# truongp-aws/neuronx-distributed-llama3_2

Hardware: AMD Instinct MI355X
Metric: tokens/sec (whole node) Llama-3-8B TP=8 bf16 training at 1/2/4/8 MI355X (higher is better)
Workload: dtype bf16

## Files before the change

### neuronx_distributed_llama3_2_amd/csrc/dense_gemm.hip

```cpp
#include "gemm_tile.h"

#include <cstdlib>
#include <type_traits>

namespace nxd {
namespace dg {

constexpr int BM = 256, BN = 256, BK = 64, NT = 512;
constexpr int REG = 16384;
constexpr int BUF = 4 * REG;
constexpr int LDS_BYTES = 2 * BUF;
constexpr int R_ALO = 0, R_AHI = REG, R_BLO = 2 * REG, R_BHI = 3 * REG;

enum Layout { LNT = 0, LTN = 1 };
enum Epi { BF16 = 0, F32_ACC = 1, F32_ATOMIC = 2 };

struct Params {
  const uint16_t* a;
  const uint16_t* b;
  void* c;
  int M, N, K;
  int64_t lda, ldb, ldc;
  int mt, nt;
  int splits;
  int k_per_split;
  int band;
};

__device__ __forceinline__ int nt_swz(int r) { return (r >> 1) & 7; }

__device__ __forceinline__ bf16x8_t frag_nt(const char* reg, int r0, int s) {
  const int l = threadIdx.x & 63, r = r0 + (l & 15), ch = (l >> 4) + 4 * s;
  return __builtin_bit_cast(bf16x8_t, *reinterpret_cast<const u32x4_t*>(reg + r * 128 + ((ch ^ nt_swz(r)) << 4)));
}
template <int L>
__device__ __forceinline__ bf16x8_t frag(const char* reg, int x0, int s) {
  if constexpr (L == LNT) return frag_nt(reg, x0, s);
  else return frag_tr16<256>(reg, x0, 32 * s);
}

__device__ __forceinline__ void wait_regions(int younger) {
  switch (younger) {
    case 5: asm volatile("s_waitcnt vmcnt(10)" ::: "memory"); break;
    case 4: asm volatile("s_waitcnt vmcnt(8)" ::: "memory"); break;
    case 3: asm volatile("s_waitcnt vmcnt(6)" ::: "memory"); break;
    case 2: asm volatile("s_waitcnt vmcnt(4)" ::: "memory"); break;
    case 1: asm volatile("s_waitcnt vmcnt(2)" ::: "memory"); break;
    default: asm volatile("s_waitcnt vmcnt(0)" ::: "memory"); break;
  }
}

template <int L, int E>
__global__ void __launch_bounds__(NT, 1) gemm_kernel(Params p) {
  __shared__ __attribute__((aligned(16))) char smem[LDS_BYTES];
  const int tiles = p.mt * p.nt;
  const int id = xcd_remap(blockIdx.x, gridDim.x);
  const int split = id / tiles;
  int rt, ct;
  band_raster(id - split * tiles, p.mt, p.nt, p.band, rt, ct);
  const int m0 = rt * BM, n0 = ct * BN;
  const int k_begin = split * p.k_per_split;
  const int k_end = min(p.K, k_begin + p.k_per_split);
  const int nk = (k_end - k_begin) / BK;

  const int wid = threadIdx.x >> 6, lane = threadIdx.x & 63;
  const int wr = wid >> 2, wc = wid & 3;

  f32x4_t acc[4][4][2];
#pragma unroll
  for (int q = 0; q < 4; ++q)
#pragma unroll
    for (int i = 0; i < 4; ++i)
#pragma unroll
      for (int j = 0; j < 2; ++j) acc[q][i][j] = f32x4_t{0.f, 0.f, 0.f, 0.f};

  const uint16_t* sa[2][2];
  const uint16_t* sb[2][2];
#pragma unroll
  for (int h = 0; h < 2; ++h)
#pragma unroll
    for (int j = 0; j < 2; ++j) {
      const int piece = 2 * wid + j;
      if constexpr (L == LNT) {
        const int pr = 8 * piece + (lane >> 3), c = (lane & 7) ^ nt_swz(pr);
        sa[h][j] = p.a + (int64_t)min(m0 + 128 * h + pr, p.M - 1) * p.lda + k_begin + 8 * c;
        sb[h][j] = p.b + (int64_t)min(n0 + 128 * h + pr, p.N - 1) * p.ldb + k_begin + 8 * c;
      } else {
        const int pr = 4 * piece + (lane >> 4), c = (lane & 15) ^ tok_swz(pr);
        sa[h][j] = p.a + (int64_t)(k_begin + pr) * p.lda + min(m0 + 128 * h + 8 * c, p.M - 8);
        sb[h][j] = p.b + (int64_t)(k_begin + pr) * p.ldb + min(n0 + 128 * h + 8 * c, p.N - 8);
      }
    }
  const int64_t adv_a = L == LNT ? (int64_t)BK : (int64_t)BK * p.lda;
  const int64_t adv_b = L == LNT ? (int64_t)BK : (int64_t)BK * p.ldb;
  const uint32_t lds0 = lds_addr(smem);

  auto issue = [&](auto rc, int s) {
    constexpr int R = decltype(rc)::value;
    if (s >= nk) return;
    const uint32_t dst = lds0 + (s & 1) * BUF + (R == 0 ? R_ALO : R == 1 ? R_BLO : R == 2 ? R_BHI : R_AHI) + wid * 2048;
    if constexpr (R == 0 || R == 3) {
      constexpr int h = R == 0 ? 0 : 1;
      const int64_t o = (int64_t)s * adv_a;
      dma16(sa[h][0] + o, __builtin_amdgcn_readfirstlane(dst));
      dma16(sa[h][1] + o, __builtin_amdgcn_readfirstlane(dst + 1024));
    } else {
      constexpr int h = R == 1 ? 0 : 1;
      const int64_t o = (int64_t)s * adv_b;
      dma16(sb[h][0] + o, __builtin_amdgcn_readfirstlane(dst));
      dma16(sb[h][1] + o, __builtin_amdgcn_readfirstlane(dst + 1024));
    }
  };
  const int last = 4 * nk - 1;
  auto wait_for = [&](int need, int max_younger = 4) {
    if (need > last) return;
    wait_regions(min(max_younger, last - need));
  };

  using I0 = std::integral_constant<int, 0>;
  using I1 = std::integral_constant<int, 1>;
  using I2 = std::integral_constant<int, 2>;
  using I3 = std::integral_constant<int, 3>;
  bf16x8_t af[4][2], blo[2][2], bhi[2][2];

  issue(I0{}, 0); issue(I1{}, 0); issue(I2{}, 0); issue(I3{}, 0); issue(I0{}, 1); issue(I1{}, 1); issue(I2{}, 1);
  wait_for(1, 5);
  barrier();
#pragma unroll
  for (int i = 0; i < 4; ++i)
#pragma unroll
    for (int s = 0; s < 2; ++s) af[i][s] = frag<L>(smem + R_ALO, wr * 64 + 16 * i, s);
#pragma unroll
  for (int j = 0; j < 2; ++j)
#pragma unroll
    for (int s = 0; s < 2; ++s) blo[j][s] = frag<L>(smem + R_BLO, wc * 32 + 16 * j, s);
  wait_for(2);
  barrier();
  for (int t = 0; t < nk; ++t) {
    const char* buf = smem + (t & 1) * BUF;
    const char* nbuf = smem + ((t + 1) & 1) * BUF;
    issue(I3{}, t + 1);
#pragma unroll
    for (int s = 0; s < 2; ++s)
#pragma unroll
      for (int i = 0; i < 4; ++i) {
#pragma unroll
        for (int j = 0; j < 2; ++j)
          acc[0][i][j] = __builtin_amdgcn_mfma_f32_16x16x32_bf16(af[i][s], blo[j][s], acc[0][i][j], 0, 0, 0);
        if (i < 2) bhi[i][s] = frag<L>(buf + R_BHI, wc * 32 + 16 * i, s);
      }
    wait_for(4 * t + 3);
    barrier();
    issue(I0{}, t + 2);
#pragma unroll
    for (int s = 0; s < 2; ++s)
#pragma unroll
      for (int i = 0; i < 4; ++i) {
#pragma unroll
        for (int j = 0; j < 2; ++j)
          acc[1][i][j] = __builtin_amdgcn_mfma_f32_16x16x32_bf16(af[i][s], bhi[j][s], acc[1][i][j], 0, 0, 0);
        af[i][s] = frag<L>(buf + R_AHI, wr * 64 + 16 * i, s);
      }
    barrier();
    issue(I1{}, t + 2);
#pragma unroll
    for (int s = 0; s < 2; ++s)
#pragma unroll
      for (int i = 0; i < 4; ++i)
#pragma unroll
        for (int j = 0; j < 2; ++j)
          acc[2][i][j] = __builtin_amdgcn_mfma_f32_16x16x32_bf16(af[i][s], bhi[j][s], acc[2][i][j], 0, 0, 0);
    wait_for(4 * t + 5);
    barrier();
    issue(I2{}, t + 2);
#pragma unroll
    for (int s = 0; s < 2; ++s)
#pragma unroll
      for (int j = 0; j < 2; ++j) {
#pragma unroll
        for (int i = 0; i < 4; ++i) {
          acc[3][i][j] = __builtin_amdgcn_mfma_f32_16x16x32_bf16(af[i][s], blo[j][s], acc[3][i][j], 0, 0, 0);
          if (j == 1) af[i][s] = frag<L>(nbuf + R_ALO, wr * 64 + 16 * i, s);
        }
        blo[j][s] = frag<L>(nbuf + R_BLO, wc * 32 + 16 * j, s);
      }
    wait_for(4 * t + 6);
    barrier();
  }
  asm volatile("s_waitcnt vmcnt(0)" ::: "memory");
  __syncthreads();

  constexpr int LD = 36;
  float* slab = reinterpret_cast<float*>(smem) + wid * (64 * LD);
  const int crow = 4 * (lane >> 4), ccol = lane & 15;
#pragma unroll
  for (int qd = 0; qd < 4; ++qd) {
    const int rh = (qd == 2 || qd == 3) ? 1 : 0, ch = (qd == 1 || qd == 2) ? 1 : 0;
#pragma unroll
    for (int i = 0; i < 4; ++i)
#pragma unroll
      for (int j = 0; j < 2; ++j)
#pragma unroll
        for (int r = 0; r < 4; ++r) slab[(16 * i + crow + r) * LD + 16 * j + ccol] = acc[qd][i][j][r];
    __builtin_amdgcn_wave_barrier();
    const int row0 = m0 + 128 * rh + 64 * wr, col0 = n0 + 128 * ch + 32 * wc;
    if constexpr (E == F32_ATOMIC) {
      const int col = col0 + (lane & 31);
      float* cp = static_cast<float*>(p.c);
#pragma unroll 8
      for (int rr = 0; rr < 32; ++rr) {
        const int lr = 2 * rr + (lane >> 5), row = row0 + lr;
        const float v = slab[lr * LD + (lane & 31)];
        if (row < p.M && col < p.N) unsafeAtomicAdd(cp + (int64_t)row * p.ldc + col, v);
      }
    } else {
#pragma unroll
      for (int ps = 0; ps < 4; ++ps) {
        const int lr = 16 * ps + (lane >> 2), c8 = 8 * (lane & 3);
        const int row = row0 + lr, col = col0 + c8;
        const f32x4_t v0 = *reinterpret_cast<const f32x4_t*>(slab + lr * LD + c8);
        const f32x4_t v1 = *reinterpret_cast<const f32x4_t*>(slab + lr * LD + c8 + 4);
        if (row < p.M && col < p.N) {
          if constexpr (E == BF16) {
            u32x4_t o;
            o[0] = pack2bf(v0[0], v0[1]); o[1] = pack2bf(v0[2], v0[3]);
            o[2] = pack2bf(v1[0], v1[1]); o[3] = pack2bf(v1[2], v1[3]);
            *reinterpret_cast<u32x4_t*>(static_cast<uint16_t*>(p.c) + (int64_t)row * p.ldc + col) = o;
          } else {
            f32x4_t* cp = reinterpret_cast<f32x4_t*>(static_cast<float*>(p.c) + (int64_t)row * p.ldc + col);
            const f32x4_t c0 = cp[0], c1 = cp[1];
            cp[0] = c0 + v0;
            cp[1] = c1 + v1;
          }
        }
      }
    }
    __builtin_amdgcn_wave_barrier();
  }
}

static int env_int(const char* name, int dflt) {
  const char* e = getenv(name);
  return e ? atoi(e) : dflt;
}

}

int dense_gemm_choose_splits(int M, int N, int K) {
  const int tiles = ceil_div(M, dg::BM) * ceil_div(N, dg::BN);
  const int steps = K / dg::BK;
  const int64_t base = (int64_t)ceil_div(tiles, 256) * steps;
  int best = 1;
  int64_t best_cost = base;
  for (int s = 2; s <= 8 && s <= steps; ++s) {
    if (steps / s < 8) break;
    const int64_t cost = (int64_t)ceil_div(tiles * s, 256) * (ceil_div(steps, s) + 6);
    if (cost * 10 < best_cost * 9 && cost < best_cost) {
      best_cost = cost;
      best = s;
    }
  }
  return best;
}

int dense_gemm_launch(int layout, int epi, const void* a, int64_t lda, const void* b, int64_t ldb, void* c, int64_t ldc,
                      int M, int N, int K, int splits, hipStream_t stream) {
  if (M <= 0 || N <= 0 || K <= 0) return 0;
  if (K % dg::BK || N % 8 || lda % 8 || ldb % 8 || ldc % 4) return -1;
  if (layout == dg::LTN && M % 8) return -1;
  if (epi == dg::BF16 && ldc % 8) return -1;
  dg::Params p{};
  p.a = static_cast<const uint16_t*>(a);
  p.b = static_cast<const uint16_t*>(b);
  p.c = c;
  p.M = M; p.N = N; p.K = K;
  p.lda = lda; p.ldb = ldb; p.ldc = ldc;
  p.mt = ceil_div(M, dg::BM);
  p.nt = ceil_div(N, dg::BN);
  const int steps = K / dg::BK;
  if (epi != dg::F32_ATOMIC) splits = 1;
  else if (splits <= 0) splits = dense_gemm_choose_splits(M, N, K);
  splits = splits < 1 ? 1 : (splits > steps ? steps : splits);
  p.k_per_split = ceil_div(steps, splits) * dg::BK;
  p.splits = ceil_div(K, p.k_per_split);
  static const int band = [] { const int v = dg::env_int("NXD_DG_BAND", 8); return v > 0 ? v : 8; }();
  p.band = band;
  const int64_t nwg = (int64_t)p.mt * p.nt * p.splits;
  if (nwg > INT32_MAX) return -2;
#define NXD_DG_LAUNCH(LY, EP) \
  hipLaunchKernelGGL((dg::gemm_kernel<LY, EP>), dim3((unsigned)nwg), dim3(dg::NT), 0, stream, p)
  if (layout == dg::LNT) {
    if (epi == dg::BF16) NXD_DG_LAUNCH(dg::LNT, dg::BF16);
    else if (epi == dg::F32_ACC) NXD_DG_LAUNCH(dg::LNT, dg::F32_ACC);
    else NXD_DG_LAUNCH(dg::LNT, dg::F32_ATOMIC);
  } else {
    if (epi == dg::BF16) NXD_DG_LAUNCH(dg::LTN, dg::BF16);
    else if (epi == dg::F32_ACC) NXD_DG_LAUNCH(dg::LTN, dg::F32_ACC);
    else NXD_DG_LAUNCH(dg::LTN, dg::F32_ATOMIC);
  }
#undef NXD_DG_LAUNCH
  return hipGetLastError() == hipSuccess ? 0 : -3;
}

}
```

### neuronx_distributed_llama3_2_amd/csrc/gemm_tile.h

```cpp
#pragma once
#include "common.h"

namespace nxd {

typedef __attribute__((address_space(3))) char lds_char_t;
typedef __attribute__((address_space(3))) short4_t lds_short4_t;

__device__ __forceinline__ uint32_t lds_addr(const char* q) { return (uint32_t)(uintptr_t)(const lds_char_t*)q; }

__device__ __forceinline__ void dma16(const void* src, uint32_t lds_dst) {
  uint32_t sv;
  asm volatile("s_mov_b32 %0, m0\n\ts_mov_b32 m0, %2\n\ts_nop 0\n\tglobal_load_lds_dwordx4 %1, off\n\ts_mov_b32 m0, %0"
               : "=&s"(sv) : "v"(src), "s"(lds_dst) : "memory");
}

__device__ __forceinline__ void barrier() {
  __builtin_amdgcn_sched_barrier(0);
  __builtin_amdgcn_s_barrier();
  __builtin_amdgcn_sched_barrier(0);
}

__device__ __forceinline__ void band_raster(int id, int rows, int cols, int band, int& r, int& c) {
  const int bnd = id / (band * cols), within = id - bnd * band * cols;
  const int h = min(band, rows - bnd * band);
  r = bnd * band + within % h;
  c = within / h;
}

__device__ __forceinline__ int tok_swz(int t) { return 2 * ((t & 3) | (((t >> 3) & 1) << 2)); }

template <int PITCH>
__device__ __forceinline__ bf16x8_t frag_tr16(const char* img, int c0, int t0) {
  const int l = threadIdx.x & 63, g = l >> 4, i = l & 15, q = i >> 2, p = i & 3;
  const int col = c0 + 4 * p, t = t0 + 8 * g + q;
  const char* b0 = img + t * PITCH + 16 * ((col >> 3) ^ tok_swz(t)) + 8 * (p & 1);
  const char* b1 = img + (t + 4) * PITCH + 16 * ((col >> 3) ^ tok_swz(t + 4)) + 8 * (p & 1);
  const short4_t lo = __builtin_amdgcn_ds_read_tr16_b64_v4i16((lds_short4_t*)b0);
  const short4_t hi = __builtin_amdgcn_ds_read_tr16_b64_v4i16((lds_short4_t*)b1);
  const short __attribute__((ext_vector_type(8))) a8 = {lo[0], lo[1], lo[2], lo[3], hi[0], hi[1], hi[2], hi[3]};
  return __builtin_bit_cast(bf16x8_t, a8);
}

}
```

### neuronx_distributed_llama3_2_amd/ops/gemm.py

```python

from __future__ import annotations

import os

import torch

from ._ext import ext, use_native

_ENABLED = os.environ.get("NXD_TUNED_GEMM", "1") == "1"


def set_overlap_safe(enabled: bool) -> None:
    if not torch.cuda.is_available():
        return
    try:
        ext().gemm_set_no_streamk(1 if enabled else 0)
    except Exception:
        pass


def _native(*t: torch.Tensor) -> bool:
    return _ENABLED and use_native(*t) and all(x.dtype in (torch.bfloat16, torch.float16) for x in t)


def linear(x: torch.Tensor, w: torch.Tensor, bias=None, out: torch.Tensor = None) -> torch.Tensor:
    shape = x.shape[:-1] + (w.shape[0],)
    if _native(x, w) and x.stride(-1) == 1:
        x2 = x.reshape(-1, x.shape[-1])
        y = out if out is not None else torch.empty(shape, dtype=x.dtype, device=x.device)
        ext().gemm(x2, w.t(), y.view(-1, w.shape[0]), None, 1.0, 0.0)
        return y + bias if bias is not None else y
    y = torch.nn.functional.linear(x, w, bias)
    if out is not None:
        out.copy_(y)
        return out
    return y


def matmul(a: torch.Tensor, b: torch.Tensor, out: torch.Tensor = None) -> torch.Tensor:
    shape = a.shape[:-1] + (b.shape[1],)
    if _native(a, b) and a.stride(-1) == 1:
        a2 = a.reshape(-1, a.shape[-1])
        y = out if out is not None else torch.empty(shape, dtype=a.dtype, device=a.device)
        ext().gemm(a2, b, y.view(-1, b.shape[1]), None, 1.0, 0.0)
        return y
    y = torch.matmul(a, b)
    if out is not None:
        out.copy_(y)
        return out
    return y


_WGRAD_BF16 = os.environ.get("NXD_WGRAD_BF16", "0") == "1"
_scratch = {}


_WGRAD_T = os.environ.get("NXD_WGRAD_T", "1")


def _use_wgrad_t(go2: torch.Tensor, x2: torch.Tensor = None, K: int = None) -> bool:
    if _WGRAD_T == "0" or _WGRAD_BF16:
        return False
    T, N = go2.shape[0], go2.shape[1]
    K = x2.shape[1] if x2 is not None else K
    if T % 8 or N % 8 or K % 8 or go2.stride(-1) != 1 or go2.stride(0) % 8:
        return False
    if x2 is not None and (x2.stride(-1) != 1 or x2.stride(0) % 8):
        return False
    return _WGRAD_T == "2" or N * K / (N + K) > 1200


_WG_KERNEL = os.environ.get("NXD_WGRAD_KERNEL", "auto")
_WG_SKINNY = 1100.0
_WG_WIDE = 16000


def _use_wgrad_kernel(mg: torch.Tensor, go2: torch.Tensor, x2: torch.Tensor, has_copy: bool = False) -> bool:
    if _WG_KERNEL == "0" or x2 is None or not _native(go2, x2) or mg.dtype != torch.float32:
        return False
    T, M = go2.shape
    N = x2.shape[1]
    if T % 32 or M % 8 or N % 8 or go2.stride(1) != 1 or x2.stride(1) != 1 or mg.stride(1) != 1:
        return False
    if go2.stride(0) % 8 or x2.stride(0) % 8 or go2.data_ptr() % 16 or x2.data_ptr() % 16:
        return False
    return _WG_KERNEL == "1" or M * N / (M + N) < _WG_SKINNY or (not has_copy and max(M, N) >= _WG_WIDE)


_DENSE_WG = os.environ.get("NXD_DENSE_WGRAD", "auto")
_DENSE_WG_SKINNY = 2200.0


def _use_dense_wgrad(mg: torch.Tensor, go2: torch.Tensor, x2, has_copy: bool) -> bool:
    if _DENSE_WG == "0" or x2 is None or not _native(go2, x2) or mg.dtype != torch.float32:
        return False
    T, M = go2.shape
    N = x2.shape[1]
    if T % 64 or M % 8 or N % 8 or go2.stride(1) != 1 or x2.stride(1) != 1 or mg.stride(1) != 1:
        return False
    if go2.stride(0) % 8 or x2.stride(0) % 8 or mg.stride(0) % 4:
        return False
    if go2.data_ptr() % 16 or x2.data_ptr() % 16 or mg.data_ptr() % 16:
        return False
    return _DENSE_WG == "1" or (not has_copy and M * N / (M + N) < _DENSE_WG_SKINNY)


def _dense_wgrad(mg: torch.Tensor, go2: torch.Tensor, x2: torch.Tensor) -> None:
    C = ext()
    T, M = go2.shape
    splits = C.dense_gemm_splits(M, x2.shape[1], T)
    C.dense_gemm(1, 1 if splits == 1 else 2, go2, x2, mg, splits)


def _wgrad_scratch(n: int, dtype, device, tag: str = "") -> torch.Tensor:
    sid = torch.cuda.current_stream(device).stream_id if torch.device(device).type == "cuda" else 0
    key = (dtype, str(device), tag, sid)
    t = _scratch.get(key)
    if t is None or t.numel() < n:
        t = _scratch[key] = torch.empty(n, dtype=dtype, device=device)
    return t[:n]


def wgrad_accumulate_(mg: torch.Tensor, go2: torch.Tensor, x2, go_t: torch.Tensor = None,
                      x_t: torch.Tensor = None) -> None:
    has_copy = go_t is not None or x_t is not None
    if _use_dense_wgrad(mg, go2, x2, has_copy):
        _dense_wgrad(mg, go2, x2)
        return
    if _use_wgrad_kernel(mg, go2, x2, has_copy=has_copy):
        ext().wgrad_gemm(mg, go2, x2, 0)
        return
    if x_t is not None and not (x_t.dim() == 2 and x_t.is_contiguous() and x_t.shape[1] == go2.shape[0]):
        x_t = None
    if x2 is None and not (x_t is not None and _native(go2, x_t) and mg.is_contiguous()
                           and _use_wgrad_t(go2, K=x_t.shape[0])):
        x2 = x_t.t().contiguous()
        x_t = None
    if x2 is None or (_native(go2, x2) and mg.is_contiguous()):
        if x2 is None or _use_wgrad_t(go2, x2):
            T, N = go2.shape[0], go2.shape[1]
            K = x_t.shape[0] if x_t is not None else x2.shape[1]
            if go_t is not None and go_t.shape == (N, T) and go_t.is_contiguous() and go_t.dtype == go2.dtype:
                gt = go_t
            else:
                gt = transpose(go2, out=_wgrad_scratch(N * T, go2.dtype, go2.device, "gt").view(N, T))
            xt = x_t if x_t is not None else transpose(x2, out=_wgrad_scratch(K * T, x2.dtype, x2.device, "xt").view(K, T))
            ext().gemm(gt, xt.t(), mg, None, 1.0, 1.0)
            return
        if _WGRAD_BF16:
            tmp = _wgrad_scratch(mg.numel(), go2.dtype, go2.device).view(mg.shape)
            ext().gemm(go2.t(), x2, tmp, None, 1.0, 0.0)
            mg.add_(tmp)
            return
        ext().gemm(go2.t(), x2, mg, None, 1.0, 1.0)
        return
    if go2.is_cuda:
        torch.addmm(mg, go2.t(), x2, out_dtype=torch.float32, out=mg)
    else:
        mg.add_(go2.t().float().matmul(x2.float()))


_DGRAD_WT = os.environ.get("NXD_DGRAD_WT", "1") == "1"
_weight_epoch = [0]


def weights_updated() -> None:
    _weight_epoch[0] += 1


def transpose(src: torch.Tensor, out: torch.Tensor = None) -> torch.Tensor:
    dst = out if out is not None else torch.empty((src.shape[1], src.shape[0]), dtype=src.dtype, device=src.device)
    if use_native(src) and src.dtype == torch.bfloat16 and src.stride(-1) == 1 and src.shape[0] % 8 == 0 \
            and src.shape[1] % 8 == 0 and src.stride(0) % 8 == 0:
        ext().transpose_bf16(src, dst)
    else:
        dst.copy_(src.t())
    return dst


def _kmajor(weight: torch.Tensor) -> torch.Tensor:
    key = (_weight_epoch[0], weight._version, weight.data_ptr())
    wt = getattr(weight, "_nxd_wt", None)
    cur = torch.cuda.current_stream(weight.device)
    if wt is None or getattr(weight, "_nxd_wt_key", None) != key:
        if wt is None or wt.shape != (weight.shape[1], weight.shape[0]):
            wt = torch.empty((weight.shape[1], weight.shape[0]), dtype=weight.dtype, device=weight.device)
        transpose(weight.detach(), out=wt)
        weight._nxd_wt = wt
        weight._nxd_wt_key = key
        weight._nxd_wt_ev = torch.cuda.Event()
        weight._nxd_wt_ev.record(cur)
        weight._nxd_wt_stream = cur.stream_id
    elif getattr(weight, "_nxd_wt_stream", cur.stream_id) != cur.stream_id:
        cur.wait_event(weight._nxd_wt_ev)
        wt.record_stream(cur)
    return wt


def dgrad(go: torch.Tensor, weight: torch.Tensor, out: torch.Tensor = None) -> torch.Tensor:
    if _DGRAD_WT and _native(go, weight) and go.stride(-1) == 1 and weight.dim() == 2 and weight.shape[0] % 8 == 0 \
            and weight.shape[1] % 8 == 0 and weight.is_contiguous():
        wt = _kmajor(weight)
        return matmul(go, wt.t(), out=out)
    return matmul(go, weight, out=out)
```

Measured before the change: 21790.

## Restructure dense GEMM main loop with SGPR-base DMA, precomputed LDS addresses, pinned schedule

Rewrites the dense GEMM mainloop into a templated per-tile routine with steady, penultimate and last modes. Global-to-LDS DMA now uses a scalar base pointer plus 32-bit per-lane offsets and sets m0 directly. LDS fragment addresses are precomputed once, and sched_group_barrier pins MFMA and ds_read interleaving. The aim is to cut VALU address arithmetic, m0 save/restore and per-iteration bounds checks so loads overlap better with MFMA. In exchange it adds a leading-dimension cap (falls back above 2^22), more complex buffer-parity bookkeeping, and hand-tuned vmcnt waits that risk correctness if miscounted.

After: 21860 (median of 6 runs). No clear change (+0.4%).

```diff
diff --git a/neuronx_distributed_llama3_2_amd/csrc/dense_gemm.hip b/neuronx_distributed_llama3_2_amd/csrc/dense_gemm.hip
--- a/neuronx_distributed_llama3_2_amd/csrc/dense_gemm.hip
+++ b/neuronx_distributed_llama3_2_amd/csrc/dense_gemm.hip
@@ -8,12 +8,14 @@
 
 constexpr int BM = 256, BN = 256, BK = 64, NT = 512;
 constexpr int REG = 16384;
-constexpr int BUF = 4 * REG;
-constexpr int LDS_BYTES = 2 * BUF;
-constexpr int R_ALO = 0, R_AHI = REG, R_BLO = 2 * REG, R_BHI = 3 * REG;
+constexpr int LDS_BYTES = 8 * REG;
+constexpr int BUF = 2 * REG;
+constexpr int R_ALO = 0, R_AHI = REG, R_BLO = 4 * REG, R_BHI = 5 * REG;
+constexpr int64_t MAX_LD = int64_t(1) << 22;
 
 enum Layout { LNT = 0, LTN = 1 };
 enum Epi { BF16 = 0, F32_ACC = 1, F32_ATOMIC = 2 };
+enum Mode { STEADY = 0, PENULT = 1, LAST = 2 };
 
 struct Params {
   const uint16_t* a;
@@ -29,26 +31,33 @@
 
 __device__ __forceinline__ int nt_swz(int r) { return (r >> 1) & 7; }
 
-__device__ __forceinline__ bf16x8_t frag_nt(const char* reg, int r0, int s) {
-  const int l = threadIdx.x & 63, r = r0 + (l & 15), ch = (l >> 4) + 4 * s;
-  return __builtin_bit_cast(bf16x8_t, *reinterpret_cast<const u32x4_t*>(reg + r * 128 + ((ch ^ nt_swz(r)) << 4)));
-}
 template <int L>
-__device__ __forceinline__ bf16x8_t frag(const char* reg, int x0, int s) {
-  if constexpr (L == LNT) return frag_nt(reg, x0, s);
-  else return frag_tr16<256>(reg, x0, 32 * s);
-}
-
-__device__ __forceinline__ void wait_regions(int younger) {
-  switch (younger) {
-    case 5: asm volatile("s_waitcnt vmcnt(10)" ::: "memory"); break;
-    case 4: asm volatile("s_waitcnt vmcnt(8)" ::: "memory"); break;
-    case 3: asm volatile("s_waitcnt vmcnt(6)" ::: "memory"); break;
-    case 2: asm volatile("s_waitcnt vmcnt(4)" ::: "memory"); break;
-    case 1: asm volatile("s_waitcnt vmcnt(2)" ::: "memory"); break;
-    default: asm volatile("s_waitcnt vmcnt(0)" ::: "memory"); break;
-  }
-}
+__device__ __forceinline__ bf16x8_t ld_frag(uint32_t a) {
+  if constexpr (L == LNT) {
+    return __builtin_bit_cast(bf16x8_t, *(const __attribute__((address_space(3))) u32x4_t*)(uintptr_t)a);
+  } else {
+    const short4_t lo = __builtin_amdgcn_ds_read_tr16_b64_v4i16((lds_short4_t*)(uintptr_t)a);
+    const short4_t hi = __builtin_amdgcn_ds_read_tr16_b64_v4i16((lds_short4_t*)(uintptr_t)(a + 1024));
+    const short __attribute__((ext_vector_type(8))) a8 = {lo[0], lo[1], lo[2], lo[3], hi[0], hi[1], hi[2], hi[3]};
+    return __builtin_bit_cast(bf16x8_t, a8);
+  }
+}
+
+template <int L>
+__device__ __forceinline__ uint32_t frag_base(int x0, int slot) {
+  const int l = threadIdx.x & 63;
+  if constexpr (L == LNT) {
+    const int r = x0 + (l & 15), ch = (l >> 4) + 4 * slot;
+    return r * 128 + ((ch ^ nt_swz(r)) << 4);
+  } else {
+    const int g = l >> 4, i = l & 15, q = i >> 2, pp = i & 3;
+    const int col = x0 + 4 * pp, t = 8 * g + q;
+    return t * 256 + 16 * ((col >> 3) ^ tok_swz(t)) + 8 * (pp & 1);
+  }
+}
+
+#define NXD_DG_MFMA 0x8
+#define NXD_DG_DSRD 0x100
 
 template <int L, int E>
 __global__ void __launch_bounds__(NT, 1) gemm_kernel(Params p) {
@@ -74,8 +83,7 @@
 #pragma unroll
       for (int j = 0; j < 2; ++j) acc[q][i][j] = f32x4_t{0.f, 0.f, 0.f, 0.f};
 
-  const uint16_t* sa[2][2];
-  const uint16_t* sb[2][2];
+  uint32_t va[2][2], vb[2][2];
 #pragma unroll
   for (int h = 0; h < 2; ++h)
 #pragma unroll
@@ -83,39 +91,34 @@
       const int piece = 2 * wid + j;
       if constexpr (L == LNT) {
         const int pr = 8 * piece + (lane >> 3), c = (lane & 7) ^ nt_swz(pr);
-        sa[h][j] = p.a + (int64_t)min(m0 + 128 * h + pr, p.M - 1) * p.lda + k_begin + 8 * c;
-        sb[h][j] = p.b + (int64_t)min(n0 + 128 * h + pr, p.N - 1) * p.ldb + k_begin + 8 * c;
+        va[h][j] = (uint32_t)(min(m0 + 128 * h + pr, p.M - 1) - m0) * (uint32_t)(2 * p.lda) + 16 * c;
+        vb[h][j] = (uint32_t)(min(n0 + 128 * h + pr, p.N - 1) - n0) * (uint32_t)(2 * p.ldb) + 16 * c;
       } else {
         const int pr = 4 * piece + (lane >> 4), c = (lane & 15) ^ tok_swz(pr);
-        sa[h][j] = p.a + (int64_t)(k_begin + pr) * p.lda + min(m0 + 128 * h + 8 * c, p.M - 8);
-        sb[h][j] = p.b + (int64_t)(k_begin + pr) * p.ldb + min(n0 + 128 * h + 8 * c, p.N - 8);
+        va[h][j] = (uint32_t)pr * (uint32_t)(2 * p.lda) + 2 * (uint32_t)min(m0 + 128 * h + 8 * c, p.M - 8);
+        vb[h][j] = (uint32_t)pr * (uint32_t)(2 * p.ldb) + 2 * (uint32_t)min(n0 + 128 * h + 8 * c, p.N - 8);
       }
-    }
-  const int64_t adv_a = L == LNT ? (int64_t)BK : (int64_t)BK * p.lda;
-  const int64_t adv_b = L == LNT ? (int64_t)BK : (int64_t)BK * p.ldb;
+      asm volatile("" : "+v"(va[h][j]), "+v"(vb[h][j]));
+    }
+  const char* pa0 = reinterpret_cast<const char*>(p.a) + 2 * (L == LNT ? (int64_t)m0 * p.lda + k_begin : (int64_t)k_begin * p.lda);
+  const char* pb0 = reinterpret_cast<const char*>(p.b) + 2 * (L == LNT ? (int64_t)n0 * p.ldb + k_begin : (int64_t)k_begin * p.ldb);
+  const int64_t adv_a = L == LNT ? (int64_t)(2 * BK) : (int64_t)(2 * BK) * p.lda;
+  const int64_t adv_b = L == LNT ? (int64_t)(2 * BK) : (int64_t)(2 * BK) * p.ldb;
   const uint32_t lds0 = lds_addr(smem);
-
-  auto issue = [&](auto rc, int s) {
-    constexpr int R = decltype(rc)::value;
-    if (s >= nk) return;
-    const uint32_t dst = lds0 + (s & 1) * BUF + (R == 0 ? R_ALO : R == 1 ? R_BLO : R == 2 ? R_BHI : R_AHI) + wid * 2048;
-    if constexpr (R == 0 || R == 3) {
-      constexpr int h = R == 0 ? 0 : 1;
-      const int64_t o = (int64_t)s * adv_a;
-      dma16(sa[h][0] + o, __builtin_amdgcn_readfirstlane(dst));
-      dma16(sa[h][1] + o, __builtin_amdgcn_readfirstlane(dst + 1024));
-    } else {
-      constexpr int h = R == 1 ? 0 : 1;
-      const int64_t o = (int64_t)s * adv_b;
-      dma16(sb[h][0] + o, __builtin_amdgcn_readfirstlane(dst));
-      dma16(sb[h][1] + o, __builtin_amdgcn_readfirstlane(dst + 1024));
-    }
-  };
-  const int last = 4 * nk - 1;
-  auto wait_for = [&](int need, int max_younger = 4) {
-    if (need > last) return;
-    wait_regions(min(max_younger, last - need));
-  };
+  const uint32_t dstw = __builtin_amdgcn_readfirstlane(lds0 + wid * 2048);
+
+  constexpr int NSA = L == LNT ? 2 : 4;
+  uint32_t ab[NSA], bb[2];
+#pragma unroll
+  for (int k = 0; k < NSA; ++k) {
+    ab[k] = lds0 + (L == LNT ? frag_base<L>(wr * 64, k) : frag_base<L>(wr * 64 + 16 * k, 0));
+    asm volatile("" : "+v"(ab[k]));
+  }
+#pragma unroll
+  for (int k = 0; k < 2; ++k) {
+    bb[k] = lds0 + R_BLO + (L == LNT ? frag_base<L>(wc * 32, k) : frag_base<L>(wc * 32 + 16 * k, 0));
+    asm volatile("" : "+v"(bb[k]));
+  }
 
   using I0 = std::integral_constant<int, 0>;
   using I1 = std::integral_constant<int, 1>;
@@ -123,70 +126,170 @@
   using I3 = std::integral_constant<int, 3>;
   bf16x8_t af[4][2], blo[2][2], bhi[2][2];
 
-  issue(I0{}, 0); issue(I1{}, 0); issue(I2{}, 0); issue(I3{}, 0); issue(I0{}, 1); issue(I1{}, 1); issue(I2{}, 1);
-  wait_for(1, 5);
+  auto fa = [&](auto par, int reg, int i, int s) {
+    constexpr int PAR = decltype(par)::value;
+    return L == LNT ? ld_frag<L>(ab[s] + PAR * BUF + reg + 2048 * i) : ld_frag<L>(ab[i] + PAR * BUF + reg + 8192 * s);
+  };
+  auto fb = [&](auto par, int reg, int j, int s) {
+    constexpr int PAR = decltype(par)::value;
+    return L == LNT ? ld_frag<L>(bb[s] + PAR * BUF + (reg - R_BLO) + 2048 * j)
+                    : ld_frag<L>(bb[j] + PAR * BUF + (reg - R_BLO) + 8192 * s);
+  };
+  auto issue = [&](auto rc, auto par, const char* src, uint32_t dstw) {
+    constexpr int R = decltype(rc)::value, PAR = decltype(par)::value;
+    constexpr int OFS = PAR * BUF + (R == 0 ? R_ALO : R == 1 ? R_BLO : R == 2 ? R_BHI : R_AHI);
+    constexpr int h = (R == 0 || R == 1) ? 0 : 1;
+    if constexpr (R == 0 || R == 3) {
+      dma16_m0<OFS>(src, va[h][0], dstw);
+      dma16_m0<OFS + 1024>(src, va[h][1], dstw);
+    } else {
+      dma16_m0<OFS>(src, vb[h][0], dstw);
+      dma16_m0<OFS + 1024>(src, vb[h][1], dstw);
+    }
+  };
+#define NXD_DG_MM(Q, I, J, S, B) \
+  acc[Q][I][J] = __builtin_amdgcn_mfma_f32_16x16x32_bf16(af[I][S], B[J][S], acc[Q][I][J], 0, 0, 0)
+#define NXD_DG_PAIR(Q, N, B)              \
+  NXD_DG_MM(Q, (N) & 3, 0, (N) >> 2, B);  \
+  NXD_DG_MM(Q, (N) & 3, 1, (N) >> 2, B)
+  constexpr int RD = L == LNT ? 1 : 2;
+#define NXD_DG_PIN(NM)                                           \
+  __builtin_amdgcn_sched_group_barrier(NXD_DG_MFMA, NM, 0);      \
+  __builtin_amdgcn_sched_group_barrier(NXD_DG_DSRD, RD, 0)
+
+  const char* pa1 = pa0 + adv_a;
+  const char* pa2 = pa1 + adv_a;
+  const char* pb2 = pb0 + 2 * adv_b;
+  auto tile = [&](auto par, auto mode) {
+    constexpr int PAR = decltype(par)::value, MODE = decltype(mode)::value;
+    using P = std::integral_constant<int, PAR>;
+    using NP = std::integral_constant<int, 1 - PAR>;
+    NXD_DG_PAIR(0, 0, blo);
+    __builtin_amdgcn_sched_barrier(0);
+    if constexpr (MODE != LAST) issue(I3{}, NP{}, pa1, dstw);
+    __builtin_amdgcn_sched_barrier(0);
+#pragma unroll
+    for (int n = 1; n < 8; ++n) {
+      NXD_DG_PAIR(0, n, blo);
+      if (n <= 4) bhi[(n - 1) & 1][(n - 1) >> 1] = fb(P{}, R_BHI, (n - 1) & 1, (n - 1) >> 1);
+    }
+    NXD_DG_PIN(2); NXD_DG_PIN(2); NXD_DG_PIN(2); NXD_DG_PIN(2);
+    __builtin_amdgcn_sched_group_barrier(NXD_DG_MFMA, 6, 0);
+    __builtin_amdgcn_sched_barrier(0);
+    if constexpr (MODE == LAST) asm volatile("s_waitcnt vmcnt(0)" ::: "memory");
+    else asm volatile("s_waitcnt vmcnt(8)" ::: "memory");
+    barrier();
+    NXD_DG_PAIR(1, 0, bhi);
+    __builtin_amdgcn_sched_barrier(0);
+    if constexpr (MODE == STEADY) issue(I0{}, P{}, pa2, dstw);
+    __builtin_amdgcn_sched_barrier(0);
+    af[0][0] = fa(P{}, R_AHI, 0, 0);
+    __builtin_amdgcn_sched_group_barrier(NXD_DG_DSRD, RD, 0);
+#pragma unroll
+    for (int n = 1; n < 8; ++n) {
+      NXD_DG_PAIR(1, n, bhi);
+      af[n & 3][n >> 2] = fa(P{}, R_AHI, n & 3, n >> 2);
+      NXD_DG_PIN(2);
+    }
+    barrier();
+    NXD_DG_PAIR(2, 0, bhi);
+    __builtin_amdgcn_sched_barrier(0);
+    if constexpr (MODE == STEADY) issue(I1{}, P{}, pb2, dstw);
+    __builtin_amdgcn_sched_barrier(0);
+#pragma unroll
+    for (int n = 1; n < 8; ++n) { NXD_DG_PAIR(2, n, bhi); }
+    __builtin_amdgcn_sched_barrier(0);
+    if constexpr (MODE == STEADY) asm volatile("s_waitcnt vmcnt(8)" ::: "memory");
+    else if constexpr (MODE == PENULT) asm volatile("s_waitcnt vmcnt(4)" ::: "memory");
+    barrier();
+    NXD_DG_MM(3, 0, 0, 0, blo);
+    NXD_DG_MM(3, 1, 0, 0, blo);
+    __builtin_amdgcn_sched_barrier(0);
+    if constexpr (MODE == STEADY) issue(I2{}, P{}, pb2, dstw);
+    __builtin_amdgcn_sched_barrier(0);
+    NXD_DG_MM(3, 2, 0, 0, blo);
+    NXD_DG_MM(3, 3, 0, 0, blo);
+    if constexpr (MODE != LAST) {
+#pragma unroll
+      for (int s = 0; s < 2; ++s) {
+        if (s == 1) {
+#pragma unroll
+          for (int i = 1; i < 4; ++i) NXD_DG_MM(3, i, 0, 1, blo);
+        }
+        blo[0][s] = fb(NP{}, R_BLO, 0, s);
+#pragma unroll
+        for (int i = 0; i < 4; ++i) {
+          NXD_DG_MM(3, i, 1, s, blo);
+          af[i][s] = fa(NP{}, R_ALO, i, s);
+        }
+        if (s == 0) NXD_DG_MM(3, 0, 0, 1, blo);
+        blo[1][s] = fb(NP{}, R_BLO, 1, s);
+      }
+      NXD_DG_PIN(2);
+      NXD_DG_PIN(1); NXD_DG_PIN(1); NXD_DG_PIN(1); NXD_DG_PIN(1); NXD_DG_PIN(1);
+      NXD_DG_PIN(3);
+      NXD_DG_PIN(1); NXD_DG_PIN(1); NXD_DG_PIN(1); NXD_DG_PIN(1);
+      __builtin_amdgcn_sched_group_barrier(NXD_DG_DSRD, RD, 0);
+      __builtin_amdgcn_sched_barrier(0);
+      if constexpr (MODE == STEADY) asm volatile("s_waitcnt vmcnt(8)" ::: "memory");
+      else asm volatile("s_waitcnt vmcnt(2)" ::: "memory");
+      barrier();
+    } else {
+#pragma unroll
+      for (int s = 0; s < 2; ++s)
+#pragma unroll
+        for (int j = 0; j < 2; ++j)
+#pragma unroll
+          for (int i = 0; i < 4; ++i)
+            if (s + j) NXD_DG_MM(3, i, j, s, blo);
+    }
+    if constexpr (MODE == STEADY) {
+      pa1 += adv_a;
+      pa2 += adv_a;
+      pb2 += adv_b;
+    }
+  };
+
+  const uint32_t pofs = (nk & 1) * BUF, qofs = BUF - pofs;
+  asm volatile("s_nop 4" ::: "memory");
+  issue(I0{}, I0{}, pa0, dstw + pofs); issue(I1{}, I0{}, pb0, dstw + pofs);
+  issue(I2{}, I0{}, pb0, dstw + pofs); issue(I3{}, I0{}, pa0, dstw + pofs);
+  if (nk >= 2) {
+    issue(I0{}, I0{}, pa1, dstw + qofs); issue(I1{}, I0{}, pb0 + adv_b, dstw + qofs);
+    issue(I2{}, I0{}, pb0 + adv_b, dstw + qofs);
+    asm volatile("s_waitcnt vmcnt(10)" ::: "memory");
+  } else {
+    asm volatile("s_waitcnt vmcnt(4)" ::: "memory");
+  }
   barrier();
 #pragma unroll
   for (int i = 0; i < 4; ++i)
 #pragma unroll
-    for (int s = 0; s < 2; ++s) af[i][s] = frag<L>(smem + R_ALO, wr * 64 + 16 * i, s);
+    for (int s = 0; s < 2; ++s)
+      af[i][s] = L == LNT ? ld_frag<L>(ab[s] + pofs + R_ALO + 2048 * i) : ld_frag<L>(ab[i] + pofs + R_ALO + 8192 * s);
 #pragma unroll
   for (int j = 0; j < 2; ++j)
 #pragma unroll
-    for (int s = 0; s < 2; ++s) blo[j][s] = frag<L>(smem + R_BLO, wc * 32 + 16 * j, s);
-  wait_for(2);
+    for (int s = 0; s < 2; ++s)
+      blo[j][s] = L == LNT ? ld_frag<L>(bb[s] + pofs + 2048 * j) : ld_frag<L>(bb[j] + pofs + 8192 * s);
+  if (nk >= 2) asm volatile("s_waitcnt vmcnt(8)" ::: "memory");
+  else asm volatile("s_waitcnt vmcnt(2)" ::: "memory");
   barrier();
-  for (int t = 0; t < nk; ++t) {
-    const char* buf = smem + (t & 1) * BUF;
-    const char* nbuf = smem + ((t + 1) & 1) * BUF;
-    issue(I3{}, t + 1);
-#pragma unroll
-    for (int s = 0; s < 2; ++s)
-#pragma unroll
-      for (int i = 0; i < 4; ++i) {
-#pragma unroll
-        for (int j = 0; j < 2; ++j)
-          acc[0][i][j] = __builtin_amdgcn_mfma_f32_16x16x32_bf16(af[i][s], blo[j][s], acc[0][i][j], 0, 0, 0);
-        if (i < 2) bhi[i][s] = frag<L>(buf + R_BHI, wc * 32 + 16 * i, s);
-      }
-    wait_for(4 * t + 3);
-    barrier();
-    issue(I0{}, t + 2);
-#pragma unroll
-    for (int s = 0; s < 2; ++s)
-#pragma unroll
-      for (int i = 0; i < 4; ++i) {
-#pragma unroll
-        for (int j = 0; j < 2; ++j)
-          acc[1][i][j] = __builtin_amdgcn_mfma_f32_16x16x32_bf16(af[i][s], bhi[j][s], acc[1][i][j], 0, 0, 0);
-        af[i][s] = frag<L>(buf + R_AHI, wr * 64 + 16 * i, s);
-      }
-    barrier();
-    issue(I1{}, t + 2);
-#pragma unroll
-    for (int s = 0; s < 2; ++s)
-#pragma unroll
-      for (int i = 0; i < 4; ++i)
-#pragma unroll
-        for (int j = 0; j < 2; ++j)
-          acc[2][i][j] = __builtin_amdgcn_mfma_f32_16x16x32_bf16(af[i][s], bhi[j][s], acc[2][i][j], 0, 0, 0);
-    wait_for(4 * t + 5);
-    barrier();
-    issue(I2{}, t + 2);
-#pragma unroll
-    for (int s = 0; s < 2; ++s)
-#pragma unroll
-      for (int j = 0; j < 2; ++j) {
-#pragma unroll
-        for (int i = 0; i < 4; ++i) {
-          acc[3][i][j] = __builtin_amdgcn_mfma_f32_16x16x32_bf16(af[i][s], blo[j][s], acc[3][i][j], 0, 0, 0);
-          if (j == 1) af[i][s] = frag<L>(nbuf + R_ALO, wr * 64 + 16 * i, s);
-        }
-        blo[j][s] = frag<L>(nbuf + R_BLO, wc * 32 + 16 * j, s);
-      }
-    wait_for(4 * t + 6);
-    barrier();
-  }
+
+  int ns = nk - 2;
+  if (ns > 0 && (ns & 1)) {
+    tile(I1{}, I0{});
+    --ns;
+  }
+  for (; ns > 0; ns -= 2) {
+    tile(I0{}, I0{});
+    tile(I1{}, I0{});
+  }
+  if (nk >= 2) tile(I0{}, I1{});
+  tile(I1{}, I2{});
+#undef NXD_DG_PIN
+#undef NXD_DG_PAIR
+#undef NXD_DG_MM
   asm volatile("s_waitcnt vmcnt(0)" ::: "memory");
   __syncthreads();
 
@@ -267,6 +370,7 @@
                       int M, int N, int K, int splits, hipStream_t stream) {
   if (M <= 0 || N <= 0 || K <= 0) return 0;
   if (K % dg::BK || N % 8 || lda % 8 || ldb % 8 || ldc % 4) return -1;
+  if (lda <= 0 || ldb <= 0 || lda > dg::MAX_LD || ldb > dg::MAX_LD) return -1;
   if (layout == dg::LTN && M % 8) return -1;
   if (epi == dg::BF16 && ldc % 8) return -1;
   dg::Params p{};
diff --git a/neuronx_distributed_llama3_2_amd/csrc/gemm_tile.h b/neuronx_distributed_llama3_2_amd/csrc/gemm_tile.h
--- a/neuronx_distributed_llama3_2_amd/csrc/gemm_tile.h
+++ b/neuronx_distributed_llama3_2_amd/csrc/gemm_tile.h
@@ -12,6 +12,12 @@
   uint32_t sv;
   asm volatile("s_mov_b32 %0, m0\n\ts_mov_b32 m0, %2\n\ts_nop 0\n\tglobal_load_lds_dwordx4 %1, off\n\ts_mov_b32 m0, %0"
                : "=&s"(sv) : "v"(src), "s"(lds_dst) : "memory");
+}
+
+template <int OFS>
+__device__ __forceinline__ void dma16_m0(const void* sbase, uint32_t voff, uint32_t lds_base) {
+  asm volatile("s_add_u32 m0, %2, %3\n\ts_nop 0\n\tglobal_load_lds_dwordx4 %0, %1"
+               : : "v"(voff), "s"(sbase), "s"(lds_base), "n"(OFS) : "memory", "scc");
 }
 
 __device__ __forceinline__ void barrier() {
diff --git a/neuronx_distributed_llama3_2_amd/ops/gemm.py b/neuronx_distributed_llama3_2_amd/ops/gemm.py
--- a/neuronx_distributed_llama3_2_amd/ops/gemm.py
+++ b/neuronx_distributed_llama3_2_amd/ops/gemm.py
@@ -87,7 +87,7 @@
     return _WG_KERNEL == "1" or M * N / (M + N) < _WG_SKINNY or (not has_copy and max(M, N) >= _WG_WIDE)
 
 
-_DENSE_WG = os.environ.get("NXD_DENSE_WGRAD", "auto")
+_DENSE_WG =os.environ.get("NXD_DENSE_WGRAD", "auto")
 _DENSE_WG_SKINNY = 2200.0
 
 
```
